# sede-open/openMCMC

Hardware: AMD Instinct MI355X
Metric: chain-updates/sec (1024 chains, 10k-node GMRF) at 1/2/4/8 GPUs vs CPU ref (higher is better)
Workload: dtype f64

## Files before the change

openmcmc_amd/csrc/omc_common.h:

```cpp
#pragma once
#include <hip/hip_runtime.h>
#include <stdint.h>

#include "omcmc_hip.h"

#define OMC_LAUNCH_LOG_MAX 64
#define OMC_SWEEP_RING_MIN 64
struct omc_ctx {
  int device;
  int dev_cus;
  int64_t n_chains;
  uint64_t seed;
  int64_t chain_offset;
  hipStream_t stream;
  bool own_stream;
  long long* d_bad_chain;
  unsigned long long* d_fallbacks;
  void* d_gamma_tab;
  unsigned long long* d_handoff;
  uint32_t run_epoch;
  int run_sweeps_per_launch;
  int run_reenter;
  int run_block_sweeps;
  int run_reenter_force;
  hipEvent_t run_ev_begin, run_ev_end;
  double* long_band; size_t long_band_bytes;
  double* long_quad; size_t long_quad_bytes;
  double* workspace;
  size_t workspace_bytes;
  void* store_ws; size_t store_ws_bytes;
  double* cov_ws; size_t cov_ws_bytes;
  void* rank_ws; size_t rank_ws_bytes;
  void* blas;
  void* blas_aux;
  hipStream_t aux_stream;
  hipEvent_t ev_fork, ev_join;
  int dense_blocked_min;
  int dense_overlap;
  double* dense_factor; size_t dense_factor_bytes;
  double* dense_winv; size_t dense_winv_bytes;
  int dense_panel_old;
  int* dense_info; size_t dense_info_bytes;
  double* slice_buf; size_t slice_buf_bytes;
// ... 373 lines not shown
```

openmcmc_amd/csrc/omc_ctx.hip:

```cpp
#include <string.h>

#include <string>

#include "omc_common.h"

static thread_local std::string g_last_error;

void omc_set_error(const char* what, hipError_t e) {
  g_last_error = std::string(what) + ": " + hipGetErrorString(e);
}

void omc_set_error_text(const char* text) { g_last_error = text; }

extern "C" {

const char* omc_last_error(void) { return g_last_error.c_str(); }

int32_t omc_abi_version(void) { return 2; }

omc_status omc_ctx_create(int32_t device, int64_t n_chains, uint64_t seed, int64_t chain_id_offset,
                          void* stream, int32_t create_stream, omc_ctx** out) {
  if (!out || n_chains <= 0 || chain_id_offset < 0) return OMC_INVALID_ARG;
  *out = nullptr;
  int count = 0;
// ... 35 lines not shown
  c->blas_aux = nullptr;
  c->aux_stream = nullptr;
  c->ev_fork = c->ev_join = nullptr;
  c->dense_overlap = 1;
  c->dense_blocked_min = 144;
  c->debug_zero_z = 0;
  c->dense_use_rocsolver = 0;
  c->gram_use_rocblas = 0;
  c->mh_use_rocblas = 0;
  c->mh_gemm_ksplit = 4;
  c->diag_algo = 0;
  c->hist_algo = 0;
  c->hist2d_algo = 0;
  c->rank_tile = 0; c->rank_chunk = 0;
  c->band_algo = 0; c->band_seg_overlap = 192; c->band_seg_count = 0; c->band_blocked_threads = 0;
  if (c->own_stream) {
    hipError_t e = hipStreamCreateWithFlags(&c->stream, hipStreamNonBlocking);
    if (e != hipSuccess) { omc_set_error("hipStreamCreate", e); delete c; return OMC_HIP_ERROR; }
  } else {
    c->stream = (hipStream_t)stream;
  }
  c->d_gamma_tab = nullptr;
  c->run_ev_begin = c->run_ev_end = nullptr;
  c->d_handoff = nullptr; c->run_epoch = 1; c->run_sweeps_per_launch = 32; c->run_reenter = 2; c->run_reenter_force = 0; c->run_block_sweeps = 0;
  hipError_t e = hipMalloc(&c->d_bad_chain, 8 * sizeof(long long));
  if (e != hipSuccess) { omc_set_error("hipMalloc", e); delete c; return OMC_HIP_ERROR; }
  c->d_fallbacks = (unsigned long long*)(c->d_bad_chain + 1);
  long long init[8] = {OMC_NO_BAD_CHAIN, 0, 0, 0, 0, 0, 0, 0};
  e = hipMemcpy(c->d_bad_chain, init, sizeof(init), hipMemcpyHostToDevice);
  if (e != hipSuccess) { omc_set_error("hipMemcpy", e); hipFree(c->d_bad_chain); delete c; return OMC_HIP_ERROR; }
  *out = c;
  return OMC_OK;
}

omc_status omc_ctx_destroy(omc_ctx* ctx) {
  if (!ctx) return OMC_INVALID_ARG;
  hipSetDevice(ctx->device);
  hipStreamSynchronize(ctx->stream);
  if (ctx->workspace) hipFree(ctx->workspace);
  if (ctx->store_ws) hipFree(ctx->store_ws);
  if (ctx->cov_ws) hipFree(ctx->cov_ws);
  if (ctx->rank_ws) hipFree(ctx->rank_ws);
  if (ctx->long_band) hipFree(ctx->long_band);
  if (ctx->long_quad) hipFree(ctx->long_quad);
  if (ctx->d_gamma_tab) hipFree(ctx->d_gamma_tab);
  if (ctx->d_handoff) hipFree(ctx->d_handoff);
  if (ctx->dense_factor) hipFree(ctx->dense_factor);
  if (ctx->dense_winv) hipFree(ctx->dense_winv);
  if (ctx->dense_info) hipFree(ctx->dense_info);
  if (ctx->slice_buf) hipFree(ctx->slice_buf);
  if (ctx->dense_tmp) hipFree(ctx->dense_tmp);
  if (ctx->rj_tmp) hipFree(ctx->rj_tmp);
  if (ctx->mh_work) hipFree(ctx->mh_work);
  if (ctx->mala.prep) hipFree(ctx->mala.prep);
  if (ctx->white.prep) hipFree(ctx->white.prep);
  if (ctx->white.a) hipFree(ctx->white.a);
  if (ctx->white.traj) hipFree(ctx->white.traj);
  if (ctx->rww.a) hipFree(ctx->rww.a);
  if (ctx->rww.mu_neg) hipFree(ctx->rww.mu_neg);
  if (ctx->rw.prep) hipFree(ctx->rw.prep);
  omc_dense_release(ctx);
  hipFree(ctx->d_bad_chain);
  if (ctx->own_stream) hipStreamDestroy(ctx->stream);
  delete ctx;
  return OMC_OK;
}

omc_status omc_ctx_synchronize(omc_ctx* ctx) {
  if (!ctx) return OMC_INVALID_ARG;
// ... 44 lines not shown
  }
  if (!strcmp(name, "band_join_fallbacks")) {
    unsigned long long v = 0;
    OMC_HIP_CHECK(hipMemcpyAsync(&v, ctx->d_fallbacks + 2, sizeof(v), hipMemcpyDeviceToHost, ctx->stream));
    OMC_HIP_CHECK(hipStreamSynchronize(ctx->stream));
    *value = (int64_t)v;
    return OMC_OK;
  }
  if (!strcmp(name, "wall_clock_khz")) {
    int khz = 0;
    OMC_HIP_CHECK(hipDeviceGetAttribute(&khz, hipDeviceAttributeWallClockRate, ctx->device));
    *value = khz;
    return OMC_OK;
  }
  if (!strcmp(name, "reenter_abi_ok")) {
    OMC_HIP_CHECK(hipSetDevice(ctx->device));
    *value = omc_reentry_probe_result(ctx);
    return OMC_OK;
  }
  if (!strcmp(name, "sweep_times_pos")) {
    *value = ctx->sweep_times_pos;
    return OMC_OK;
  }
  if (!strcmp(name, "tridiag_join_fallbacks")) {
    unsigned long long v = 0;
    OMC_HIP_CHECK(hipMemcpyAsync(&v, ctx->d_fallbacks, sizeof(v), hipMemcpyDeviceToHost, ctx->stream));
    OMC_HIP_CHECK(hipStreamSynchronize(ctx->stream));
    *value = (int64_t)v;
    return OMC_OK;
  }
  return OMC_INVALID_ARG;
}

omc_status omc_ctx_launch_log(omc_ctx* ctx, double* out, int64_t cap, int64_t* n_launches) {
  if (!ctx || !n_launches || cap < 0 || (cap > 0 && !out)) return OMC_INVALID_ARG;
  *n_launches = ctx->launch_log_total;
  const int64_t m = ctx->launch_log_n < cap ? ctx->launch_log_n : cap;
  for (int64_t i = 0; i < m; ++i) {
    const omc_ctx::LaunchRec& r = ctx->launch_log[i];
    out[5 * i] = r.t_begin; out[5 * i + 1] = r.t_end; out[5 * i + 2] = (double)r.n_sweeps; out[5 * i + 3] = (double)r.form;
    out[5 * i + 4] = (double)r.ring_pos;
  }
  return OMC_OK;
}

omc_status omc_ctx_set_option(omc_ctx* ctx, const char* name, int64_t value) {
// ... 23 lines not shown
    ctx->run_reenter = (int)value;
    ctx->run_reenter_force = 1;
    return OMC_OK;
  }
  if (!strcmp(name, "tridiag_quad_skip")) {
    if (value < 0 || value > 15) return OMC_INVALID_ARG;
    ctx->tridiag_quad_skip = (int)value;
    return OMC_OK;
  }
  if (!strcmp(name, "tridiag_perturb_ppb")) {
    if (value < 0 || value > 1000000000) return OMC_INVALID_ARG;
    ctx->tridiag_perturb_ppb = (int)value;
    return OMC_OK;
  }
  if (!strcmp(name, "tridiag_newton_max")) {
    if (value < 0 || value > 64) return OMC_INVALID_ARG;
    ctx->tridiag_newton_max = (int)value;
    return OMC_OK;
  }
  if (!strcmp(name, "tridiag_generic")) {
    ctx->tridiag_generic = value != 0;
    return OMC_OK;
  }
  if (!strcmp(name, "band_algo")) {
    if (value < 0 || value > 3) return OMC_INVALID_ARG;
    ctx->band_algo = (int)value;
    return OMC_OK;
  }
  if (!strcmp(name, "diag_algo")) {
    if (value < 0 || value > 2) return OMC_INVALID_ARG;
    ctx->diag_algo = (int)value;
    return OMC_OK;
  }
  if (!strcmp(name, "hist_algo")) {
    if (value < 0 || value > 1) return OMC_INVALID_ARG;
    ctx->hist_algo = (int)value;
    return OMC_OK;
  }
  if (!strcmp(name, "hist2d_algo")) {
    if (value < 0 || value > 3) return OMC_INVALID_ARG;
    ctx->hist2d_algo = (int)value;
    return OMC_OK;
  }
  if (!strcmp(name, "rank_tile")) {
    if (value != 0 && (value < 64 || value > 8192 || (value & (value - 1)))) return OMC_INVALID_ARG;
    ctx->rank_tile = (int)value;
// ... 84 lines not shown
```

openmcmc_amd/csrc/omc_tridiag.hip:

```cpp
#include <math.h>
#include <time.h>

#include "omc_common.h"
#include "omc_tridiag_args.h"
#include "omc_tridiag_epilogue.h"

__global__ void __launch_bounds__(64) k_tridiag_serial(TriArgs A) {
  const int64_t c = (int64_t)blockIdx.x * blockDim.x + threadIdx.x;
  if (c >= A.C) return;
  const int nt = A.T.n_terms;
  const int64_t n = A.n;
  double sc[OMC_MAX_TERMS];
  _Pragma("unroll") for (int k = 0; k < OMC_MAX_TERMS; ++k) if (k < nt) sc[k] = A.T.scale[k] ? A.T.scale[k][c] : 1.0;
  double* lw = A.work + c * n;
  double* xo = A.x + c * A.ld_x;
  const int64_t gc = A.chain_offset + c;
  bool bad = false;
  double lp = 0.0, bprev = 0.0, u = 0.0, logdet = 0.0, zodd = 0.0;
  for (int64_t i = 0; i < n; ++i) {
    double av = 0.0, bv = 0.0, rv = 0.0;
    _Pragma("unroll") for (int k = 0; k < OMC_MAX_TERMS; ++k) if (k < nt) {
      av = fma(sc[k], A.T.diag[k] ? A.T.diag[k][i] : 1.0, av);
      if (A.T.off[k] && i < n - 1) bv = fma(sc[k], A.T.off[k][i], bv);
      if (A.T.rhs[k]) rv = fma(sc[k], A.T.rhs[k][i], rv);
// ... 73 lines not shown
  const bool no_private = private_size == 0u && (rsrc2 & 1u) == 0u && (props & (1u << 11)) == 0u;
  const bool wave64 = (props & (1u << 10)) == 0u;
  return user_sgprs && system_sgprs && no_private && wave64 && preload == 0u;
}

static int g_reentry_ok = -1;
static bool reentry_abi_ok(omc_ctx* ctx) {
  if (g_reentry_ok >= 0) return g_reentry_ok != 0;
  uint32_t* d = nullptr;
  uint32_t h[6] = {~0u, ~0u, ~0u, ~0u, ~0u, ~0u};
  bool ok = hipMalloc(&d, sizeof(h)) == hipSuccess;
  if (ok) {
    hipLaunchKernelGGL(k_reentry_probe, dim3(1), dim3(64), 0, ctx->stream, d);
    ok = hipMemcpyAsync(h, d, sizeof(h), hipMemcpyDeviceToHost, ctx->stream) == hipSuccess &&
         hipStreamSynchronize(ctx->stream) == hipSuccess;
    hipFree(d);
  }
  ok = ok && reentry_descriptor_ok(h[0], h[1], h[2]) && reentry_descriptor_ok(h[3], h[4], h[5]);
  g_reentry_ok = ok ? 1 : 0;
  if (!ok) omc_set_error_text("omc_gmrf_run: the kernel descriptor does not match the restart's entry state; self-restarting workgroups are off");
  return ok;
}
int omc_reentry_probe_result(omc_ctx* ctx) { return reentry_abi_ok(ctx) ? 1 : 0; }

__global__ void k_tridiag_matvec(int64_t n, const double* diag, const double* off, const double* v, double* out) {
  for (int64_t i = (int64_t)blockIdx.x * blockDim.x + threadIdx.x; i < n; i += (int64_t)gridDim.x * blockDim.x) {
    double t = (diag ? diag[i] : 1.0) * v[i];
    if (off) {
      if (i > 0) t = fma(off[i - 1], v[i - 1], t);
      if (i < n - 1) t = fma(off[i], v[i + 1], t);
    }
    out[i] = t;
  }
}

__global__ void __launch_bounds__(256) k_tridiag_matvec_chain(int64_t n, const double* diag, const double* off, const double* v,
                                                              int64_t ld_v, const double* scale, double* out, int64_t ld_o,
                                                              int accumulate) {
  const int64_t c = blockIdx.y;
  const double s = scale ? scale[c] : 1.0;
  const double* vc = v + c * ld_v;
  for (int64_t i = (int64_t)blockIdx.x * blockDim.x + threadIdx.x; i < n; i += (int64_t)gridDim.x * blockDim.x) {
    double t = (diag ? diag[i] : 1.0) * vc[i];
    if (off) {
      if (i > 0) t = fma(off[i - 1], vc[i - 1], t);
      if (i < n - 1) t = fma(off[i], vc[i + 1], t);
// ... 132 lines not shown
    const bool on = k < t->n_terms;
    d->diag[k] = on ? t->diag[k] : nullptr;
    d->off[k] = on ? t->off[k] : nullptr;
    d->rhs[k] = on ? t->rhs[k] : nullptr;
    d->center[k] = on ? t->center[k] : nullptr;
    d->scale[k] = on ? t->scale[k] : nullptr;
  }
  if (cc) {
    *cc = CentreChain{};
    for (int k = 0; k < t->n_terms; ++k)
      if (t->center_chain[k]) {
        cc->k = cc->v ? -1 : k;
        cc->v = t->center_chain[k];
      }
    cc->ld = t->ld_center_chain;
  }
  return true;
}
static bool has_center_chain(const CentreChain& cc) { return cc.v != nullptr; }

static void args_defaults(omc_ctx* ctx, TriArgs* A, int64_t n) {
  A->T = TermsDev{};
  A->cc = CentreChain{};
  A->n = n; A->C = ctx->n_chains; A->chain_offset = ctx->chain_offset;
  A->rhs_chain = nullptr; A->ld_rhs = 0;
  A->z = nullptr; A->ld_z = 0; A->zero_z = 0;
  A->key = omc_make_key(ctx->seed, 0, OMC_RNG_NORMAL);
  A->x = nullptr; A->ld_x = 0; A->quad = nullptr; A->logdet = nullptr;
  A->bad = ctx->d_bad_chain;
  A->fallbacks = ctx->d_fallbacks;
  A->newton_max = ctx->tridiag_newton_max;
  A->perturb_start = ctx->tridiag_perturb_ppb * 1e-9;
  A->work = nullptr;
  A->fused = 0;
  A->stamps = ctx->stamps;
  A->sweep_times = nullptr; A->sweep_times_cap = 0; A->sweep_times_pos = 0;
  A->log_post = nullptr;
  A->gb_dev = nullptr; A->gdraw_dev = nullptr;
  A->n_sweeps = 0; A->reenter = 0; A->block_sweeps = 0; A->early_draws = 0; A->epoch = 0; A->seed = ctx->seed; A->handoff = nullptr; A->timeouts = ctx->d_fallbacks + 1;
  for (int k = 0; k < OMC_MAX_TERMS; ++k) A->gdraw[k] = 0;
  for (int i = 0; i < OMC_RUN_MAX; ++i) { A->rec[i].draw = 0; A->rec[i].x = nullptr; A->rec[i].log_post = nullptr; A->rec[i].slot_off = -1; }
  for (int k = 0; k < OMC_MAX_TERMS; ++k) {
    A->gb[k].enabled = 0; A->gb[k].a0 = A->gb[k].b0 = A->gb[k].half_npos = A->gb[k].lnorm = 0.0;
    A->gb[k].g_inject = nullptr; A->gb[k].store = nullptr; A->gb[k].scale_out = nullptr;
    A->gb[k].logdet_unscaled = nullptr; A->gb[k].key = A->key;
  }
// ... 327 lines not shown
    if (!ctx->d_handoff) {
      const size_t bytes = (size_t)C * OMC_HANDOFF_WORDS * sizeof(unsigned long long);
      OMC_HIP_CHECK(hipMalloc(&ctx->d_handoff, bytes));
      OMC_HIP_CHECK(hipMemsetAsync(ctx->d_handoff, 0, bytes, ctx->stream));
      ctx->run_epoch = 1;
    }
    A.handoff = ctx->d_handoff;
    A.ld_x = ld_x;
    A.zero_z = ctx->debug_zero_z;
    A.fused = 1;
    const int per = ctx->run_sweeps_per_launch < OMC_RUN_MAX ? ctx->run_sweeps_per_launch : OMC_RUN_MAX;
    const int dev_cus = ctx->dev_cus;
    const int64_t rounds = (C + dev_cus - 1) / dev_cus;
    const bool whole_rounds = C >= dev_cus && (double)C >= 0.95 * (double)(rounds * dev_cus);
    A.reenter = (whole_rounds || ctx->run_reenter_force) ? ctx->run_reenter : 0;
    if (!takes_specialised(ctx, A.T, n) || has_center_chain(A.cc)) A.reenter = 0;
    if (A.reenter && per > 1 && !reentry_abi_ok(ctx)) A.reenter = 0;
    if (A.reenter && C * (int64_t)per >= ((int64_t)1 << 26)) A.reenter = 0;
    A.early_draws = (A.reenter == 0 && 2 * C <= dev_cus && !has_center_chain(A.cc)) ? 1 : 0;
    const int64_t stored_per_launch_max = (A.reenter == 0 && n_slots < per) ? n_slots : per;
    ctx->launch_log_n = 0; ctx->launch_log_total = 0;
    const bool clock_on = ctx->sweep_times && ctx->sweep_times_cap >= OMC_SWEEP_RING_MIN;
    if (ctx->run_ev_begin) OMC_HIP_CHECK(hipEventRecord(ctx->run_ev_begin, ctx->stream));
    for (int64_t t0 = 0; t0 < total;) {
      int k_sw = (int)(total - t0 < per ? total - t0 : per);
      if (stored_per_launch_max < per) {
        int64_t stored_seen = 0;
        for (int i = 0; i < k_sw; ++i) {
          const int64_t t = t0 + i;
          if (t >= burn && ((t - burn + 1) % n_thin == 0) && ++stored_seen > stored_per_launch_max) { k_sw = i; break; }
        }
      }
      for (int i = 0; i < k_sw; ++i) {
        const int64_t t = t0 + i;
        const bool stored = t >= burn && ((t - burn + 1) % n_thin == 0);
        const int64_t it = stored ? (t - burn + 1) / n_thin - 1 : 0;
        const int64_t slot = (first_slot + it) % n_slots;
        A.rec[i].draw = draw_index0 + (uint64_t)t * draws_per_sweep;
        A.rec[i].x = stored ? x_store + slot * x_slot_stride : (t == total - 1 ? scratch_x : nullptr);
        A.rec[i].log_post = (stored && log_post_store) ? log_post_store + slot * C : nullptr;
        A.rec[i].slot_off = stored ? slot * C : -1;
      }
      A.n_sweeps = k_sw;
      A.block_sweeps = k_sw;
      if (A.reenter && ctx->run_block_sweeps > 0 && ctx->run_block_sweeps < k_sw) A.block_sweeps = ctx->run_block_sweeps;
      A.epoch = ctx->run_epoch;
      ctx->run_epoch += (uint32_t)k_sw;
      A.key = omc_make_key(ctx->seed, A.rec[0].draw, OMC_RNG_NORMAL);
      A.x = A.rec[0].x;
      A.log_post = A.rec[0].log_post;
      if (clock_on) {
        A.sweep_times = ctx->sweep_times; A.sweep_times_cap = ctx->sweep_times_cap; A.sweep_times_pos = ctx->sweep_times_pos;
      }
      const double t_begin = omc_host_clock();
      omc_status st = launch_tridiag(ctx, A);
      if (st != OMC_OK) return st;
      if (ctx->launch_log_n < OMC_LAUNCH_LOG_MAX) {
        omc_ctx::LaunchRec& r = ctx->launch_log[ctx->launch_log_n++];
        r.t_begin = t_begin; r.t_end = omc_host_clock(); r.n_sweeps = k_sw; r.form = A.reenter;
        r.ring_pos = clock_on ? ctx->sweep_times_pos : -1;
      }
      ctx->launch_log_total++;
      if (clock_on) ctx->sweep_times_pos = (ctx->sweep_times_pos + k_sw) % ctx->sweep_times_cap;
      t0 += k_sw;
    }
    if (ctx->run_ev_end) OMC_HIP_CHECK(hipEventRecord(ctx->run_ev_end, ctx->stream));
    return OMC_OK;
  }
  ctx->launch_log_n = 0; ctx->launch_log_total = 0;
  for (int64_t t = 0; t < total; ++t) {
    const bool stored = t >= burn && ((t - burn + 1) % n_thin == 0);
    const int64_t i = stored ? (t - burn + 1) / n_thin - 1 : 0;
    const int64_t slot = (first_slot + i) % n_slots;
    const uint64_t base = draw_index0 + (uint64_t)t * draws_per_sweep;
    for (int k = 0; k < terms->n_terms && k < OMC_MAX_TERMS; ++k) {
      b[k] = blocks[k];
      b[k].draw_index = base + blocks[k].draw_index;
      b[k].store = (stored && blocks[k].store) ? blocks[k].store + slot * C : nullptr;
    }
    const double t_begin = omc_host_clock();
    omc_status st = omc_gmrf_sweep(ctx, n, terms, b, nullptr, 0, nullptr, 0, base,
                                   stored ? x_store + slot * x_slot_stride : scratch_x, ld_x,
                                   (stored && log_post_store) ? log_post_store + slot * C : nullptr);
    if (st != OMC_OK) return st;
    if (ctx->launch_log_n < OMC_LAUNCH_LOG_MAX) {
      omc_ctx::LaunchRec& r = ctx->launch_log[ctx->launch_log_n++];
      r.t_begin = t_begin; r.t_end = omc_host_clock(); r.n_sweeps = 1; r.form = 0; r.ring_pos = -1;
    }
    ctx->launch_log_total++;
  }
  return OMC_OK;
}
// ... 77 lines not shown
```

openmcmc_amd/csrc/omc_tridiag_args.h:

```cpp
#pragma once
#include "omc_common.h"

struct TermsDev {
  int n_terms;
  const double* diag[OMC_MAX_TERMS];
  const double* off[OMC_MAX_TERMS];
  const double* rhs[OMC_MAX_TERMS];
  const double* center[OMC_MAX_TERMS];
  const double* scale[OMC_MAX_TERMS];
};
struct CentreChain {
  const double* v;
  int64_t ld;
  int quad_skip;
  int k;
};

struct GammaDev {
  int enabled;
  double a0, b0, half_npos;
  double lnorm;
  const double* g_inject;
  double* store;
  double* scale_out;
// ... 24 lines not shown
  double perturb_start;
  int newton_max;
  unsigned long long* fallbacks;
  double* work;
  unsigned long long* stamps;
  int fused;
  GammaDev gb[OMC_MAX_TERMS];
  const GammaDev* gb_dev;
  const unsigned long long* gdraw_dev;
  double* log_post;
  int n_sweeps;
  int reenter;
  int block_sweeps;
  int early_draws;
  uint32_t epoch;
  uint64_t seed;
  uint64_t gdraw[OMC_MAX_TERMS];
  unsigned long long* handoff;
  unsigned long long* timeouts;
  unsigned long long* sweep_times;
  int64_t sweep_times_cap, sweep_times_pos;
  SweepRec rec[OMC_RUN_MAX];
  CentreChain cc;
};

__device__ __forceinline__ bool run_mode(const TriArgs& A) { return A.n_sweeps > 0; }
__device__ __forceinline__ omc_rng_key sweep_gamma_key(const TriArgs& A, int sw, const GammaDev& g, uint64_t gd) {
  return run_mode(A) ? omc_make_key(A.seed, A.rec[sw].draw + gd, OMC_RNG_GAMMA) : g.key;
}
__device__ __forceinline__ double* sweep_gamma_store(const TriArgs& A, int sw, const GammaDev& g) {
  if (!run_mode(A)) return g.store;
  const int64_t off = A.rec[sw].slot_off;
  return (g.store && off >= 0) ? g.store + off : nullptr;
}
__device__ __forceinline__ double* sweep_log_post(const TriArgs& A, int sw) { return run_mode(A) ? A.rec[sw].log_post : A.log_post; }
```

openmcmc_amd/csrc/omc_tridiag_seg.h:

```cpp
#pragma once
#include "omc_tridiag_epilogue.h"
#include "omc_tridiag_scan.h"
#include "omc_tridiag_tile.h"

#ifndef OMC_PARK_OFF
#define OMC_PARK_OFF 1
#endif
#ifndef OMC_PARK_DIAG
#define OMC_PARK_DIAG 1
#endif
#ifndef OMC_SHIFT_PARK_C
#define OMC_SHIFT_PARK_C 1
#endif
#ifndef OMC_PREFETCH_QUAD
#define OMC_PREFETCH_QUAD 1
#endif
#ifndef OMC_WHATIF_NOSTORE
#define OMC_WHATIF_NOSTORE 0
#endif
#ifndef OMC_WHATIF_NOQLOAD
#define OMC_WHATIF_NOQLOAD 0
#endif
#ifndef OMC_NO_STAMPS
#define OMC_NO_STAMPS 0
// ... 74 lines not shown
    }
    c = blk;
    s = threadIdx.x;
    geo.chain0 = c;
  } else {
    const int cpw = 64 / G;
    geo.chain0 = ((int64_t)blockIdx.x * nw + wave) * cpw;
    c = geo.chain0 + lane / G;
    s = lane % G;
  }
  double* tile = lds_tile[wave];
  const double* trow = tile + (MULTI ? lane : s) * (M + 1);
  double* crow = tile + lane * (M + 1);
  const int lbase = TileMap<M>::lane_base(lane);
  const int pos = MULTI ? lane : s;
  const bool chain_ok = c < A.C;
  const int64_t cc = chain_ok ? c : 0;
  const int64_t n = A.n;
  const int64_t i0 = (int64_t)s * M;
  const int nt = (SMO) ? 2 : A.T.n_terms;
  const int wave_u = __builtin_amdgcn_readfirstlane(wave);
  const int r0 = TM::lane_col(lane);
  double* tl = tile + lbase;

  double sc[OMC_MAX_TERMS];
  const bool handed = MULTI && sw > 0;
  const bool hand_lds = SIG == 1 && A.reenter != 0 && restarted;
  if (SIG == 1 && A.reenter != 0 && !restarted && threadIdx.x < 2 * OMC_MAX_TERMS)
    __hip_atomic_store(lds_hand + threadIdx.x, 0ull, __ATOMIC_RELAXED, __HIP_MEMORY_SCOPE_WORKGROUP);
  unsigned long long hw[2 * OMC_MAX_TERMS];
  auto load_hand_global = [&](int k) __attribute__((always_inline)) {
    const unsigned long long* h = A.handoff + cc * OMC_HANDOFF_WORDS + 2 * k;
    hw[2 * k] = __hip_atomic_load(h, __ATOMIC_RELAXED, __HIP_MEMORY_SCOPE_AGENT);
    hw[2 * k + 1] = __hip_atomic_load(h + 1, __ATOMIC_RELAXED, __HIP_MEMORY_SCOPE_AGENT);
  };
  auto load_hand_lds = [&](int k) __attribute__((always_inline)) {
    hw[2 * k] = __hip_atomic_load(lds_hand + 2 * k, __ATOMIC_RELAXED, __HIP_MEMORY_SCOPE_WORKGROUP);
    hw[2 * k + 1] = __hip_atomic_load(lds_hand + 2 * k + 1, __ATOMIC_RELAXED, __HIP_MEMORY_SCOPE_WORKGROUP);
  };
#pragma unroll
  for (int k = 0; k < OMC_MAX_TERMS; ++k) {
    sc[k] = 1.0;
    hw[2 * k] = hw[2 * k + 1] = 0ull;
    if (k < nt && A.T.scale[k]) {
      if (handed && A.gb[k].enabled) {
        if (!hand_lds) load_hand_global(k);
// ... 87 lines not shown
    bool f = false;
    const double g = sweep_gamma_draws_wave<MULTI && !SMO>(A, c, lane, &f, sw);
    lds_g[lane] = f ? -g : g;
  }

  OMC_STAMP(1);
  const int64_t gc = A.chain_offset + cc;
  const uint32_t blk0 = (uint32_t)(i0 >> 1);
  const bool gen_z = !A.z && !A.zero_z;
  auto park_pair = [&](int jb) __attribute__((always_inline)) {
    double z0, z1;
    omc_normal_pair(omc_rng_block(nkey_f(), gc, blk0 + (uint32_t)jb), z0, z1);
    lds_z[wave][2 * jb][lane] = z0;
    lds_z[wave][2 * jb + 1][lane] = z1;
  };
  auto park_pair_over_load = [&](int jb, double (&v)[M], const double* base, int nvalid) __attribute__((always_inline)) {
    double z0, z1;
    if (nvalid == 64 * M) draws_over_load<M, true>(nkey_f(), gc, blk0 + (uint32_t)jb, z0, z1, v, base, lane, nvalid);
    else draws_over_load<M, false>(nkey_f(), gc, blk0 + (uint32_t)jb, z0, z1, v, base, lane, nvalid);
    lds_z[wave][2 * jb][lane] = z0;
    lds_z[wave][2 * jb + 1][lane] = z1;
  };
  const double* const vPark = (SHIFT && OMC_SHIFT_PARK_C) ? vSh : vPo;
  const bool park_off = OMC_PARK_OFF && SMO && gen_z && (A.quad || A.fused) &&
                        wave_valid<M>(wave_u, (int)n - ((SHIFT && OMC_SHIFT_PARK_C) ? 0 : 1)) == 64 * M &&
                        (reinterpret_cast<uintptr_t>(vPark) & 15u) == 0;
  const bool park_diag = OMC_PARK_DIAG && SMO && (A.quad || A.fused) && wave_valid<M>(wave_u, (int)n) == 64 * M &&
                         (reinterpret_cast<uintptr_t>(vPd) & 15u) == 0;
  const int e_nv = EARLY ? wave_valid<M>(wave_u, (int)n) : 0, e_nvo = EARLY ? wave_valid<M>(wave_u, (int)n - 1) : 0;
  const bool e_partial = EARLY && (A.quad || A.fused) && e_nv > 0 && e_nv < 64 * M && !(A.rhs_chain && chain_ok);
  const bool park_off_p = OMC_PARK_OFF && e_partial && gen_z && e_nvo >= 2 && (reinterpret_cast<uintptr_t>(vPo) & 15u) == 0;
  double e_edge_o = 0.0;

  const bool early1 = !EARLY && SMO && gen_z && A.early_draws != 0;
  const bool gen_late = gen_z && !EARLY && !early1;
  if constexpr (SMO && !EARLY) {
    if (early1) {
#pragma unroll
      for (int jb = 0; jb < NZB; ++jb) park_pair(jb);
    }
  }
  double pre[M];
  double Rrow[EARLY ? M : 1], ebm1_raw = 0.0, ezl0 = 0.0, ezl1 = 0.0;
  if constexpr (EARLY) {
    if (gen_z) {
#pragma unroll
      for (int jb = 0; jb < NZB; ++jb) park_pair(jb);
    }
    if (epi_wave && chain_ok) {
      bool f = false;
      const double g = sweep_gamma_draws_wave(A, c, lane, &f, sw);
// ... 16 lines not shown
      wave_lds_fence();
    };
    if (!(A.rhs_chain && chain_ok)) {
      stage(vIr + wbase, env);
#pragma unroll
      for (int j = 0; j < M; ++j) Rrow[j] = crow[j];
    }
    stage(vPo + wbase, envo);
#pragma unroll
    for (int j = 0; j < M; ++j) Y[j] = crow[j];
    stage(vPd + wbase, env);
    __builtin_amdgcn_sched_barrier(0);
    if (handed) {
      if (threadIdx.x < 2 * OMC_MAX_TERMS) __hip_atomic_store(lds_hand + threadIdx.x, 0ull, __ATOMIC_RELAXED, __HIP_MEMORY_SCOPE_WORKGROUP);
      lds_barrier();
    }
  }
  auto fill_draws = [&](int jb) {
    if constexpr (PARKZ && !SMO) {
      if (gen_z && jb < NZB) park_pair(jb);
    }
  };
  double bm1 = 0.0;
  if constexpr (SMO) {
    const int wbase = wave_u * 64 * M;
    const int nv = wave_valid<M>(wave_u, (int)n), nvo = wave_valid<M>(wave_u, (int)n - 1);
    auto vec_and_draws = [&](double (&v)[M], const double* base, int nvalid, int jb) {
      if (gen_late && jb < NZB) park_pair_over_load(jb, v, base, nvalid);
      else coal_load<M>(v, base, lane, nvalid);
      __builtin_amdgcn_sched_barrier(0);
    };
    {
      double po[M];
      double bm1_raw;
      if constexpr (EARLY) {
        bm1_raw = ebm1_raw;
      } else {
        bm1_raw = vPo[(i0 > 0 && i0 < n) ? i0 - 1 : 0];
        vec_and_draws(po, vPo + wbase, nvo, 0);
      }
      take_scales();
      if (SIG == 1 && A.reenter == 2 && handed && hand_lds && wave_u == 1 && chain_ok && any_handed_f()) {
        double* const lp_prev = A.rec[sw - 1].log_post;
        if (lp_prev) {
          const int k = lane >> 4;
          const double sk = (k == 0) ? sc[0] : ((k == 1) ? sc[1] : ((k == 2) ? sc[2] : sc[3]));
          const double qk = (k < nt) ? __hip_atomic_load(lds_q + (k < nt ? k : 0), __ATOMIC_RELAXED, __HIP_MEMORY_SCOPE_WORKGROUP) : 0.0;
          double ldk = 0.0;
          _Pragma("unroll") for (int t = 0; t < OMC_MAX_TERMS; ++t)
            if (t < nt && k == t && A.gb[t].logdet_unscaled) ldk = A.gb[t].logdet_unscaled[0];
          sweep_log_post_wave(A, c, lane, (k < nt) ? sk : 1.0, qk, ldk, lp_prev);
        }
      }
      sP = p_first ? sc[0] : sc[1];
      sI = p_first ? sc[1] : sc[0];
      if constexpr (EARLY) {
#pragma unroll
        for (int j = 0; j < M; ++j) Y[j] *= sP;
        if (!(A.rhs_chain && chain_ok)) {
#pragma unroll
          for (int j = 0; j < M; ++j) Rrow[j] *= sI;
        }
      } else {
        wave_lds_fence();
#pragma unroll
        for (int t = 0; t < M; ++t) *TM::elem(tl, r0, t) = sP * po[t];
        wave_lds_fence();
      }
      bm1 = (i0 > 0 && i0 < n) ? sP * bm1_raw : 0.0;
    }
    if constexpr (EARLY) {
      OMC_STAMP(2);
    } else {
      double pd[M];
      vec_and_draws(pd, vPd + wbase, nv, 1);
#pragma unroll
      for (int j = 0; j < M; ++j) Y[j] = crow[j];
      OMC_STAMP(2);
      wave_lds_fence();
      if (nv == 64 * M) {
#pragma unroll
        for (int t = 0; t < M; ++t) *TM::elem(tl, r0, t) = fma(sP, pd[t], sI);
      } else {
#pragma unroll
        for (int t = 0; t < M; ++t) *TM::elem(tl, r0, t) = (lane + 64 * t < nv) ? fma(sP, pd[t], sI) : 1.0;
      }
      wave_lds_fence();
    }
  } else {
    take_scales();
    if (MULTI) tile_fill_comb_wg<M, COMB_OFF>(tile, lane, wave, lbase, A, sc, chain_ok, cc, [&](int b) { if (b == 0) fill_draws(0); });
    else tile_fill_comb<M, MULTI, COMB_OFF>(tile, geo, A, sc);
#pragma unroll
    for (int j = 0; j < M; ++j) Y[j] = crow[j];
    if (i0 > 0 && i0 < n)
      _Pragma("unroll") for (int k = 0; k < OMC_MAX_TERMS; ++k) if (k < nt)
        if (A.T.off[k]) bm1 = fma(sc[k], A.T.off[k][i0 - 1], bm1);
    OMC_STAMP(2);
    if (MULTI) tile_fill_comb_wg<M, COMB_DIAG>(tile, lane, wave, lbase, A, sc, chain_ok, cc, [&](int b) { if (b == 0) fill_draws(1); });
    else tile_fill_comb<M, MULTI, COMB_DIAG>(tile, geo, A, sc);
  }
  const double* arow = crow;
  auto a_at = [&](int j) -> double {
    if constexpr (EARLY) return fma(sP, arow[j], sI);
    else return arow[j];
  };

  OMC_STAMP(3);
  double Dst;
  double Dnext0 = 0.0;
  {
    Mob m{1.0, 0.0, 0.0, 1.0};
    double bp = bm1;
#pragma unroll
    for (int j = 0; j < M; ++j) {
      const double b2 = bp * bp, aj = a_at(j);
      const double na = fma(aj, m.a, -b2 * m.c), nb = fma(aj, m.b, -b2 * m.d);
      m.c = m.a; m.d = m.b; m.a = na; m.b = nb;
      bp = Y[j];
      if ((j & 7) == 7) {
        const int ex = -__builtin_amdgcn_frexp_exp(m.a);
        m = Mob{ldexp(m.a, ex), ldexp(m.b, ex), ldexp(m.c, ex), ldexp(m.d, ex)};
      }
    }
    m = mob_rescale(m);
    OMC_STAMP(4);
    const Mob idm{1.0, 0.0, 0.0, 1.0};
    const Mob E = MULTI ? excl_scan_wg<Mob, false, true>(m, idm, lds_mob, lane, wave, nw, lds_mob2)
                        : excl_scan<Mob, false>(m, idm, pos, Wd, false, lds_mob, wave, nw);
    Dst = (E.a + E.b) / (E.c + E.d);
    if (A.perturb_start != 0.0 && s > 0) Dst *= 1.0 + A.perturb_start;
    if (MULTI) {
      const Mob inc = compose(m, E);
      Dnext0 = (inc.a + inc.b) * fast_rcp(inc.c + inc.d);
      if (A.perturb_start != 0.0) Dnext0 *= 1.0 + A.perturb_start;
    }
  }

  OMC_STAMP(5);
  bool bad = false;
  double lin = 0.0;
  auto pivot_pass = [&]() -> double {
    wave_lds_fence();
    const double rst = fast_rcp(Dst);
    lin = bm1 * rst;
    double lp = lin, bprev = bm1, Dend = Dst;
    bool badp = false;
#pragma unroll
    for (int j = 0; j < M; ++j) {
      const double D = fma(-lp, bprev, a_at(j));
      badp |= !(D > 0.0);
      const double r = fast_rcp(D);
      W[j] = r;
      bprev = Y[j];
      lp = bprev * r;
      Dend = D;
    }
    bad = badp;
    return Dend;
  };
  double Dend = pivot_pass();
  bool settled = false;
  if (MULTI) {
    const bool has_next = i0 + M < n;
    const int need = (has_next && fabs(Dend - Dnext0) > OMC_NEWTON_TOL * fabs(Dnext0)) ? 1 : 0;
    settled = !any_wg(need, lds_any, lane, wave, nw);
  }
  for (int it = 0; !settled; ++it) {
    double J = lin * lin;
#pragma unroll
    for (int j = 0; j + 1 < M; ++j) {
      const double l = Y[j] * W[j];
      J *= l * l;
    }
    double Dp = Dend, Jp = J;
    if (MULTI) prev_lane2_wg(Dp, Jp, Dst, 0.0, lds_x[it & 1], lane, wave, nw);
    else prev_lane2<false>(Dp, Jp, Dst, 0.0, pos, Wd, lds_x[0], wave);
    const bool joined = (s > 0 && i0 < n);
    const double e = joined ? (Dp - Dst) : 0.0;
    if (!joined) Jp = 0.0;
    const int need = (fabs(e) > OMC_NEWTON_TOL * fabs(Dst)) ? 1 : 0;
    const int any = MULTI ? __syncthreads_or(need) : (__ballot(need) != 0ull);
// ... 82 lines not shown
    }
  }
  if (rhs_done) {
  } else if (MULTI) {
    if constexpr (SMO) tile_fill_comb_wg<M, COMB_RHS, false>(tile, lane, wave, lbase, A, sc, chain_ok, cc);
    else tile_fill_comb_wg<M, COMB_RHS, true>(tile, lane, wave, lbase, A, sc, chain_ok, cc, [&](int b) { fill_draws(2 + b); });
    if constexpr (EARLY) {
#pragma unroll
      for (int j = 0; j < M; ++j) Rrow[j] = crow[j];
    }
  } else {
    tile_fill_comb<M, MULTI, COMB_RHS>(tile, geo, A, sc);
  }
  constexpr bool PFQ = SMO && OMC_PREFETCH_QUAD;
  constexpr int PFQ_LOADS = M;
  static_assert(!PFQ || PFQ_LOADS <= 15, "vmcnt immediate");
  double qcp[PFQ ? M : 1];
  double qcc[SHIFT ? M : 1];
  bool pfq = false;
  int pfq_behind = 0;
  auto issue_pfq = [&]() {
    if constexpr (PFQ) {
      const bool wq = A.quad || A.fused;
      pfq = wq && park_off && wave_valid<M>(wave_u, (int)n) == 64 * M;
      __builtin_amdgcn_sched_barrier(0);
      if constexpr (EARLY) {
        if (e_partial) {
          const int wbase = wave_u * 64 * M;
#pragma unroll
          for (int t = 0; t < M; ++t) qcp[t] = (lane + 64 * t < e_nv) ? (vIc + wbase)[(unsigned)(lane + 64 * t)] : 0.0;
        }
      }
      if (pfq) {
        const int wbase = wave_u * 64 * M;
        if (!SHIFT || vIc) {
#pragma unroll
          for (int t = 0; t < M; ++t) qcp[t] = (vIc + wbase)[(unsigned)(lane + 64 * t)];
          pfq_behind += M;
        } else {
#pragma unroll
          for (int t = 0; t < M; ++t) qcp[t] = 0.0;
        }
      }
      __builtin_amdgcn_sched_barrier(0);
    }
  };
  OMC_STAMP(8);
// ... 49 lines not shown
          }
        }
        if constexpr (EARLY) {
          z0 = crow[M]; z1 = ezl1;
        } else {
          omc_normal_pair(omc_rng_block(nkey_f(), gc, blk0 + (uint32_t)(j >> 1)), z0, z1);
        }
      }
      u = fma(-lp, u, r_at(j));
      W[j] = fma(u, W[j], z0 * fast_sqrt(W[j]));
      lp = Y[j];
      u = fma(-lp, u, r_at(j + 1));
      W[j + 1] = fma(u, W[j + 1], z1 * fast_sqrt(W[j + 1]));
      lp = Y[j + 1];
      if (!(PARKZ && (j >> 1) < NZB - 1)) __builtin_amdgcn_sched_barrier(0);
    }
  }

  OMC_STAMP(10);
  const bool want_quad = A.quad || A.fused;
  double aPd = 0.0;
  double eqd[EARLY ? M : 1];
  const bool diag_staged = EARLY && !(A.rhs_chain && chain_ok);
  if constexpr (SMO) {
    if (park_diag && !diag_staged) {
      lds_reads_done();
#pragma unroll
      for (int k = 0; k < (64 * M) / 128; ++k)
        __builtin_amdgcn_global_load_lds((const __attribute__((address_space(1))) void*)(vPd + wave_u * 64 * M + 128 * k + 2 * lane),
                                         (__attribute__((address_space(3))) void*)(tile + 128 * k), 16, 0, 0);
    }
  }
  issue_pfq();
  double xnext;
  {
    Aff f{0.0, 1.0};
#pragma unroll
    for (int j = M - 1; j >= 0; --j) {
      f.p = fma(-Y[j], f.p, W[j]);
      f.q = -Y[j] * f.q;
    }
    xnext = (MULTI ? excl_scan_wg<Aff, true>(f, Aff{0.0, 1.0}, lds_aff[3], lane, wave, nw)
                   : excl_scan<Aff, false>(f, Aff{0.0, 1.0}, pos, Wd, true, lds_aff[0], wave, nw)).p;
    double x = xnext;
    OMC_STAMP(11);
    if constexpr (EARLY) {
      if (e_partial) {
        wave_lds_fence();
#pragma unroll
        for (int t = 0; t < M; ++t) eqd[t] = *TM::elem(tl, r0, t);
      }
    }
    if (SMO && park_diag) {
      if (!diag_staged) {
        if (PFQ && pfq_behind >= PFQ_LOADS) __builtin_amdgcn_s_waitcnt(0x0F70 | PFQ_LOADS);
        else __builtin_amdgcn_s_waitcnt(0x0F70);
      }
      wave_lds_fence();
      const double* drow = diag_staged ? crow : tile + lane * M;
#pragma unroll
      for (int j = M - 1; j >= 0; --j) {
        x = fma(-Y[j], x, W[j]);
        W[j] = x;
        aPd = fma(drow[j] * x, x, aPd);
      }
    } else {
#pragma unroll
      for (int j = M - 1; j >= 0; --j) {
        x = fma(-Y[j], x, W[j]);
        W[j] = x;
      }
    }
  }
  OMC_STAMP(12);
  double qsum[OMC_MAX_TERMS] = {0, 0, 0, 0};
  double my_scale = 1.0, my_logdet = 0.0;
  if (MULTI) {
    wave_lds_fence();
#pragma unroll
    for (int j = 0; j < M; ++j) crow[j] = W[j];
    if (lane == 63) tile[64 * (M + 1)] = xnext;
    wave_lds_fence();
    double acc[OMC_MAX_TERMS] = {0, 0, 0, 0};
    if (epi_wave) {
      _Pragma("unroll") for (int k = 0; k < OMC_MAX_TERMS; ++k) if (k < nt && (lane >> 4) == k) {
        if (A.T.scale[k]) my_scale = handed ? sc[k] : A.T.scale[k][cc];
        if constexpr (SMO) {
          if (sweep_log_post(A, sw) && A.gb[k].logdet_unscaled) my_logdet = A.gb[k].logdet_unscaled[0];
        }
      }
      if constexpr (!SMO) {
        const double* const ldp = ((lane >> 4) < nt) ? A.gb_dev[lane >> 4].logdet_unscaled : nullptr;
        if (sweep_log_post(A, sw) && ldp) my_logdet = ldp[0];
      }
    }
    if constexpr (SMO) {
      if (!EARLY && epi_wave && chain_ok) {
        bool f = false;
        const double g = sweep_gamma_draws_wave(A, c, lane, &f, sw);
        lds_g[lane] = f ? -g : g;
      }
      const int nv = wave_valid<M>(wave_u, (int)n);
      double qc[M], qd[M], qo[M];
      {
        const int wbase = wave_u * 64 * M;
        const int nvq = want_quad ? nv : 0, nvo = want_quad ? wave_valid<M>(wave_u, (int)n - 1) : 0;
        {
          if (park_off && SHIFT && OMC_SHIFT_PARK_C) {
            const double* zf = &lds_z[wave][0][0];
            coal_load<M>(qo, vPo + wbase, lane, nvo);
            __builtin_amdgcn_s_waitcnt(0x0F70 | M);
            wave_lds_fence();
#pragma unroll
            for (int t = 0; t < M; ++t)
              if (t < 2 * NZB) qcc[t] = zf[64 * t + lane];
#pragma unroll
            for (int t = 0; t < M; ++t) {
              if (t < 2 * NZB) continue;
              qcc[t] = (vSh + wbase)[(unsigned)(lane + 64 * t)];
            }
          } else if (park_off) {
            const double* zf = &lds_z[wave][0][0];
            __builtin_amdgcn_s_waitcnt(0x0F70);
            wave_lds_fence();
#pragma unroll
            for (int t = 0; t < M; ++t)
              if (t < 2 * NZB) qo[t] = zf[64 * t + lane];
#pragma unroll
            for (int t = 0; t < M; ++t) {
              if (t < 2 * NZB) continue;
              qo[t] = OMC_WHATIF_NOQLOAD ? 0.25 : (vPo + wbase)[(unsigned)(lane + 64 * t)];
// ... 217 lines not shown
```

Measured before the change: 13.08 million.

## Detect constant tridiagonal slices and skip per-element diag/off loads

Adds a pre-pass kernel that checks whether each wave-sized slice of the precision diagonal and off-diagonal is constant, and records the flags and values in a small table. In the specialised single-term segment kernel, waves whose slice is constant use the scalar value instead of loading the vector from global memory or staging it through LDS. This targets memory traffic and LDS work in the factor and quad passes. The cost is an extra launch per run plus added branches and register pressure, and the fast path only applies when the inputs happen to have constant runs.

Result: no change. 13.21 million, median of 6 (+0.9%).

```diff
diff --git a/openmcmc_amd/csrc/omc_common.h b/openmcmc_amd/csrc/omc_common.h
--- a/openmcmc_amd/csrc/omc_common.h
+++ b/openmcmc_amd/csrc/omc_common.h
@@ -5,6 +5,10 @@
 #include "omcmc_hip.h"
 
 #define OMC_LAUNCH_LOG_MAX 64
+#define OMC_SLICE_WORDS 4
+#define OMC_SLICE_MAX 16
+#define OMC_SLICE_OFF 1ull
+#define OMC_SLICE_DIAG 2ull
 #define OMC_SWEEP_RING_MIN 64
 struct omc_ctx {
   int device;
@@ -19,6 +23,9 @@
   void* d_gamma_tab;
   unsigned long long* d_handoff;
   uint32_t run_epoch;
+  unsigned long long* d_slices;
+  int run_slices;
+  int run_slices_n;
   int run_sweeps_per_launch;
   int run_reenter;
   int run_block_sweeps;
diff --git a/openmcmc_amd/csrc/omc_ctx.hip b/openmcmc_amd/csrc/omc_ctx.hip
--- a/openmcmc_amd/csrc/omc_ctx.hip
+++ b/openmcmc_amd/csrc/omc_ctx.hip
@@ -81,6 +81,7 @@
   }
   c->d_gamma_tab = nullptr;
   c->run_ev_begin = c->run_ev_end = nullptr;
+  c->d_slices = nullptr; c->run_slices = 1; c->run_slices_n = 0;
   c->d_handoff = nullptr; c->run_epoch = 1; c->run_sweeps_per_launch = 32; c->run_reenter = 2; c->run_reenter_force = 0; c->run_block_sweeps = 0;
   hipError_t e = hipMalloc(&c->d_bad_chain, 8 * sizeof(long long));
   if (e != hipSuccess) { omc_set_error("hipMalloc", e); delete c; return OMC_HIP_ERROR; }
@@ -104,6 +105,7 @@
   if (ctx->long_quad) hipFree(ctx->long_quad);
   if (ctx->d_gamma_tab) hipFree(ctx->d_gamma_tab);
   if (ctx->d_handoff) hipFree(ctx->d_handoff);
+  if (ctx->d_slices) hipFree(ctx->d_slices);
   if (ctx->dense_factor) hipFree(ctx->dense_factor);
   if (ctx->dense_winv) hipFree(ctx->dense_winv);
   if (ctx->dense_info) hipFree(ctx->dense_info);
@@ -194,6 +196,17 @@
     *value = ctx->sweep_times_pos;
     return OMC_OK;
   }
+  if (!strcmp(name, "tridiag_const_slices")) {
+    unsigned long long w[OMC_SLICE_MAX * OMC_SLICE_WORDS];
+    const int m = ctx->run_slices_n;
+    *value = 0;
+    if (m <= 0 || !ctx->d_slices) return OMC_OK;
+    OMC_HIP_CHECK(hipMemcpyAsync(w, ctx->d_slices, (size_t)m * OMC_SLICE_WORDS * sizeof(w[0]), hipMemcpyDeviceToHost, ctx->stream));
+    OMC_HIP_CHECK(hipStreamSynchronize(ctx->stream));
+    for (int i = 0; i < m; ++i)
+      *value += (int64_t)((w[OMC_SLICE_WORDS * i] & OMC_SLICE_OFF) != 0ull) + (int64_t)((w[OMC_SLICE_WORDS * i] & OMC_SLICE_DIAG) != 0ull);
+    return OMC_OK;
+  }
   if (!strcmp(name, "tridiag_join_fallbacks")) {
     unsigned long long v = 0;
     OMC_HIP_CHECK(hipMemcpyAsync(&v, ctx->d_fallbacks, sizeof(v), hipMemcpyDeviceToHost, ctx->stream));
@@ -263,6 +276,10 @@
     ctx->tridiag_generic = value != 0;
     return OMC_OK;
   }
+  if (!strcmp(name, "tridiag_slices")) {
+    ctx->run_slices = value != 0;
+    return OMC_OK;
+  }
   if (!strcmp(name, "band_algo")) {
     if (value < 0 || value > 3) return OMC_INVALID_ARG;
     ctx->band_algo = (int)value;
diff --git a/openmcmc_amd/csrc/omc_tridiag.hip b/openmcmc_amd/csrc/omc_tridiag.hip
--- a/openmcmc_amd/csrc/omc_tridiag.hip
+++ b/openmcmc_amd/csrc/omc_tridiag.hip
@@ -119,6 +119,29 @@
   return ok;
 }
 int omc_reentry_probe_result(omc_ctx* ctx) { return reentry_abi_ok(ctx) ? 1 : 0; }
+
+__global__ void __launch_bounds__(256) k_tridiag_slices(int64_t n, int slice, const double* diag, const double* off,
+                                                        unsigned long long* tab) {
+  const int64_t base = (int64_t)blockIdx.x * slice;
+  const bool in_d = base + slice <= n, in_o = base + slice <= n - 1;
+  const unsigned long long* const d = reinterpret_cast<const unsigned long long*>(diag) + base;
+  const unsigned long long* const o = reinterpret_cast<const unsigned long long*>(off) + base;
+  const unsigned long long d0 = in_d ? d[0] : 0ull, o0 = in_o ? o[0] : 0ull;
+  int same_d = in_d ? 1 : 0, same_o = in_o ? 1 : 0;
+  for (int i = threadIdx.x; i < slice; i += blockDim.x) {
+    if (in_d) same_d &= (d[i] == d0) ? 1 : 0;
+    if (in_o) same_o &= (o[i] == o0) ? 1 : 0;
+  }
+  same_d = __syncthreads_and(same_d);
+  same_o = __syncthreads_and(same_o);
+  if (threadIdx.x == 0) {
+    unsigned long long* const e = tab + (int64_t)blockIdx.x * OMC_SLICE_WORDS;
+    e[0] = (same_o ? OMC_SLICE_OFF : 0ull) | (same_d ? OMC_SLICE_DIAG : 0ull);
+    e[1] = o0;
+    e[2] = d0;
+    e[3] = 0ull;
+  }
+}
 
 __global__ void k_tridiag_matvec(int64_t n, const double* diag, const double* off, const double* v, double* out) {
   for (int64_t i = (int64_t)blockIdx.x * blockDim.x + threadIdx.x; i < n; i += (int64_t)gridDim.x * blockDim.x) {
@@ -297,6 +320,7 @@
 static void args_defaults(omc_ctx* ctx, TriArgs* A, int64_t n) {
   A->T = TermsDev{};
   A->cc = CentreChain{};
+  A->slices = nullptr;
   A->n = n; A->C = ctx->n_chains; A->chain_offset = ctx->chain_offset;
   A->rhs_chain = nullptr; A->ld_rhs = 0;
   A->z = nullptr; A->ld_z = 0; A->zero_z = 0;
@@ -670,6 +694,21 @@
     ctx->launch_log_n = 0; ctx->launch_log_total = 0;
     const bool clock_on = ctx->sweep_times && ctx->sweep_times_cap >= OMC_SWEEP_RING_MIN;
     if (ctx->run_ev_begin) OMC_HIP_CHECK(hipEventRecord(ctx->run_ev_begin, ctx->stream));
+    ctx->run_slices_n = 0;
+    if (ctx->run_slices && total >= 2 && takes_specialised(ctx, A.T, n) && !has_center_chain(A.cc) &&
+        !(A.early_draws && !A.reenter && !A.zero_z)) {
+      const int seg = ctx->tridiag_seg ? ctx->tridiag_seg : auto_seg(n);
+      const int n_sl = (int)((n + 64 * seg - 1) / (64 * seg));
+      if (n_sl <= OMC_SLICE_MAX) {
+        if (!ctx->d_slices) OMC_HIP_CHECK(hipMalloc(&ctx->d_slices, (size_t)OMC_SLICE_MAX * OMC_SLICE_WORDS * sizeof(unsigned long long)));
+        const bool p_first = A.T.diag[0] != nullptr;
+        hipLaunchKernelGGL(k_tridiag_slices, dim3((unsigned)n_sl), dim3(256), 0, ctx->stream, n, 64 * seg,
+                           p_first ? A.T.diag[0] : A.T.diag[1], p_first ? A.T.off[0] : A.T.off[1], ctx->d_slices);
+        OMC_HIP_CHECK(hipGetLastError());
+        A.slices = ctx->d_slices;
+        ctx->run_slices_n = n_sl;
+      }
+    }
     for (int64_t t0 = 0; t0 < total;) {
       int k_sw = (int)(total - t0 < per ? total - t0 : per);
       if (stored_per_launch_max < per) {
@@ -716,6 +755,7 @@
     return OMC_OK;
   }
   ctx->launch_log_n = 0; ctx->launch_log_total = 0;
+  ctx->run_slices_n = 0;
   for (int64_t t = 0; t < total; ++t) {
     const bool stored = t >= burn && ((t - burn + 1) % n_thin == 0);
     const int64_t i = stored ? (t - burn + 1) / n_thin - 1 : 0;
diff --git a/openmcmc_amd/csrc/omc_tridiag_args.h b/openmcmc_amd/csrc/omc_tridiag_args.h
--- a/openmcmc_amd/csrc/omc_tridiag_args.h
+++ b/openmcmc_amd/csrc/omc_tridiag_args.h
@@ -70,6 +70,7 @@
   int64_t sweep_times_cap, sweep_times_pos;
   SweepRec rec[OMC_RUN_MAX];
   CentreChain cc;
+  const unsigned long long* slices;
 };
 
 __device__ __forceinline__ bool run_mode(const TriArgs& A) { return A.n_sweeps > 0; }
diff --git a/openmcmc_amd/csrc/omc_tridiag_seg.h b/openmcmc_amd/csrc/omc_tridiag_seg.h
--- a/openmcmc_amd/csrc/omc_tridiag_seg.h
+++ b/openmcmc_amd/csrc/omc_tridiag_seg.h
@@ -1,4 +1,6 @@
 #pragma once
+#include <type_traits>
+
 #include "omc_tridiag_epilogue.h"
 #include "omc_tridiag_scan.h"
 #include "omc_tridiag_tile.h"
@@ -120,6 +122,16 @@
   const int wave_u = __builtin_amdgcn_readfirstlane(wave);
   const int r0 = TM::lane_col(lane);
   double* tl = tile + lbase;
+  unsigned long long sl_flags = 0ull;
+  double off0 = 0.0, d0 = 0.0;
+  if constexpr (SIG == 1) {
+    if (A.slices) {
+      const auto* st = (const __attribute__((address_space(4))) unsigned long long*)(uintptr_t)A.slices + OMC_SLICE_WORDS * wave_u;
+      sl_flags = st[0];
+      off0 = __longlong_as_double((long long)st[1]);
+      d0 = __longlong_as_double((long long)st[2]);
+    }
+  }
 
   double sc[OMC_MAX_TERMS];
   const bool handed = MULTI && sw > 0;
@@ -253,11 +265,14 @@
     lds_z[wave][2 * jb + 1][lane] = z1;
   };
   const double* const vPark = (SHIFT && OMC_SHIFT_PARK_C) ? vSh : vPo;
-  const bool park_off = OMC_PARK_OFF && SMO && gen_z && (A.quad || A.fused) &&
-                        wave_valid<M>(wave_u, (int)n - ((SHIFT && OMC_SHIFT_PARK_C) ? 0 : 1)) == 64 * M &&
-                        (reinterpret_cast<uintptr_t>(vPark) & 15u) == 0;
+  const bool c_off = SIG == 1 && (sl_flags & OMC_SLICE_OFF) != 0ull && wave_valid<M>(wave_u, (int)n - 1) == 64 * M;
+  const bool park_off_any = OMC_PARK_OFF && SMO && gen_z && (A.quad || A.fused) &&
+                            wave_valid<M>(wave_u, (int)n - ((SHIFT && OMC_SHIFT_PARK_C) ? 0 : 1)) == 64 * M &&
+                            (reinterpret_cast<uintptr_t>(vPark) & 15u) == 0;
+  const bool park_off = park_off_any && !c_off;
   const bool park_diag = OMC_PARK_DIAG && SMO && (A.quad || A.fused) && wave_valid<M>(wave_u, (int)n) == 64 * M &&
                          (reinterpret_cast<uintptr_t>(vPd) & 15u) == 0;
+  const bool c_diag = SIG == 1 && (sl_flags & OMC_SLICE_DIAG) != 0ull && park_diag;
   const int e_nv = EARLY ? wave_valid<M>(wave_u, (int)n) : 0, e_nvo = EARLY ? wave_valid<M>(wave_u, (int)n - 1) : 0;
   const bool e_partial = EARLY && (A.quad || A.fused) && e_nv > 0 && e_nv < 64 * M && !(A.rhs_chain && chain_ok);
   const bool park_off_p = OMC_PARK_OFF && e_partial && gen_z && e_nvo >= 2 && (reinterpret_cast<uintptr_t>(vPo) & 15u) == 0;
@@ -320,12 +335,17 @@
     }
   };
   double bm1 = 0.0;
+  double a0 = 0.0;
   if constexpr (SMO) {
     const int wbase = wave_u * 64 * M;
     const int nv = wave_valid<M>(wave_u, (int)n), nvo = wave_valid<M>(wave_u, (int)n - 1);
     auto vec_and_draws = [&](double (&v)[M], const double* base, int nvalid, int jb) {
       if (gen_late && jb < NZB) park_pair_over_load(jb, v, base, nvalid);
       else coal_load<M>(v, base, lane, nvalid);
+      __builtin_amdgcn_sched_barrier(0);
+    };
+    auto draws_alone = [&](int jb) {
+      if (gen_late && jb < NZB) park_pair(jb);
       __builtin_amdgcn_sched_barrier(0);
     };
     {
@@ -359,7 +379,7 @@
 #pragma unroll
           for (int j = 0; j < M; ++j) Rrow[j] *= sI;
         }
-      } else {
+      } else if (!c_off) {
         wave_lds_fence();
 #pragma unroll
         for (int t = 0; t < M; ++t) *TM::elem(tl, r0, t) = sP * po[t];
@@ -371,12 +391,20 @@
       OMC_STAMP(2);
     } else {
       double pd[M];
-      vec_and_draws(pd, vPd + wbase, nv, 1);
-#pragma unroll
-      for (int j = 0; j < M; ++j) Y[j] = crow[j];
+      if (c_diag) draws_alone(1);
+      else vec_and_draws(pd, vPd + wbase, nv, 1);
+      if (c_off) {
+#pragma unroll
+        for (int j = 0; j < M; ++j) Y[j] = sP * off0;
+      } else {
+#pragma unroll
+        for (int j = 0; j < M; ++j) Y[j] = crow[j];
+      }
       OMC_STAMP(2);
       wave_lds_fence();
-      if (nv == 64 * M) {
+      if (c_diag) {
+        a0 = fma(sP, d0, sI);
+      } else if (nv == 64 * M) {
 #pragma unroll
         for (int t = 0; t < M; ++t) *TM::elem(tl, r0, t) = fma(sP, pd[t], sI);
       } else {
@@ -399,28 +427,40 @@
     else tile_fill_comb<M, MULTI, COMB_DIAG>(tile, geo, A, sc);
   }
   const double* arow = crow;
-  auto a_at = [&](int j) -> double {
-    if constexpr (EARLY) return fma(sP, arow[j], sI);
+  auto a_at = [&](int j, auto cd) -> double {
+    if constexpr (decltype(cd)::value) return a0;
+    else if constexpr (EARLY) return fma(sP, arow[j], sI);
     else return arow[j];
+  };
+  using CdYes = std::integral_constant<bool, true>;
+  using CdNo = std::integral_constant<bool, false>;
+  auto by_diag = [&](auto f) {
+    if constexpr (SIG == 1) {
+      if (c_diag) return f(CdYes{});
+    }
+    return f(CdNo{});
   };
 
   OMC_STAMP(3);
   double Dst;
   double Dnext0 = 0.0;
   {
-    Mob m{1.0, 0.0, 0.0, 1.0};
-    double bp = bm1;
-#pragma unroll
-    for (int j = 0; j < M; ++j) {
-      const double b2 = bp * bp, aj = a_at(j);
-      const double na = fma(aj, m.a, -b2 * m.c), nb = fma(aj, m.b, -b2 * m.d);
-      m.c = m.a; m.d = m.b; m.a = na; m.b = nb;
-      bp = Y[j];
-      if ((j & 7) == 7) {
-        const int ex = -__builtin_amdgcn_frexp_exp(m.a);
-        m = Mob{ldexp(m.a, ex), ldexp(m.b, ex), ldexp(m.c, ex), ldexp(m.d, ex)};
-      }
-    }
+    Mob m = by_diag([&](auto cd) {
+      Mob m{1.0, 0.0, 0.0, 1.0};
+      double bp = bm1;
+#pragma unroll
+      for (int j = 0; j < M; ++j) {
+        const double b2 = bp * bp, aj = a_at(j, cd);
+        const double na = fma(aj, m.a, -b2 * m.c), nb = fma(aj, m.b, -b2 * m.d);
+        m.c = m.a; m.d = m.b; m.a = na; m.b = nb;
+        bp = Y[j];
+        if ((j & 7) == 7) {
+          const int ex = -__builtin_amdgcn_frexp_exp(m.a);
+          m = Mob{ldexp(m.a, ex), ldexp(m.b, ex), ldexp(m.c, ex), ldexp(m.d, ex)};
+        }
+      }
+      return m;
+    });
     m = mob_rescale(m);
     OMC_STAMP(4);
     const Mob idm{1.0, 0.0, 0.0, 1.0};
@@ -442,20 +482,22 @@
     wave_lds_fence();
     const double rst = fast_rcp(Dst);
     lin = bm1 * rst;
-    double lp = lin, bprev = bm1, Dend = Dst;
-    bool badp = false;
-#pragma unroll
-    for (int j = 0; j < M; ++j) {
-      const double D = fma(-lp, bprev, a_at(j));
-      badp |= !(D > 0.0);
-      const double r = fast_rcp(D);
-      W[j] = r;
-      bprev = Y[j];
-      lp = bprev * r;
-      Dend = D;
-    }
-    bad = badp;
-    return Dend;
+    return by_diag([&](auto cd) {
+      double lp = lin, bprev = bm1, Dend = Dst;
+      bool badp = false;
+#pragma unroll
+      for (int j = 0; j < M; ++j) {
+        const double D = fma(-lp, bprev, a_at(j, cd));
+        badp |= !(D > 0.0);
+        const double r = fast_rcp(D);
+        W[j] = r;
+        bprev = Y[j];
+        lp = bprev * r;
+        Dend = D;
+      }
+      bad = badp;
+      return Dend;
+    });
   };
   double Dend = pivot_pass();
   bool settled = false;
@@ -584,7 +626,7 @@
   auto issue_pfq = [&]() {
     if constexpr (PFQ) {
       const bool wq = A.quad || A.fused;
-      pfq = wq && park_off && wave_valid<M>(wave_u, (int)n) == 64 * M;
+      pfq = wq && park_off_any && wave_valid<M>(wave_u, (int)n) == 64 * M;
       __builtin_amdgcn_sched_barrier(0);
       if constexpr (EARLY) {
         if (e_partial) {
@@ -680,13 +722,15 @@
   double aPd = 0.0;
   double eqd[EARLY ? M : 1];
   const bool diag_staged = EARLY && !(A.rhs_chain && chain_ok);
+  int diag_xfers = 0;
   if constexpr (SMO) {
-    if (park_diag && !diag_staged) {
+    if (park_diag && !diag_staged && !c_diag) {
       lds_reads_done();
 #pragma unroll
       for (int k = 0; k < (64 * M) / 128; ++k)
         __builtin_amdgcn_global_load_lds((const __attribute__((address_space(1))) void*)(vPd + wave_u * 64 * M + 128 * k + 2 * lane),
                                          (__attribute__((address_space(3))) void*)(tile + 128 * k), 16, 0, 0);
+      diag_xfers += (64 * M) / 128;
     }
   }
   issue_pfq();
@@ -710,17 +754,26 @@
       }
     }
     if (SMO && park_diag) {
-      if (!diag_staged) {
+      if (diag_xfers > 0) {
         if (PFQ && pfq_behind >= PFQ_LOADS) __builtin_amdgcn_s_waitcnt(0x0F70 | PFQ_LOADS);
         else __builtin_amdgcn_s_waitcnt(0x0F70);
       }
       wave_lds_fence();
-      const double* drow = diag_staged ? crow : tile + lane * M;
-#pragma unroll
-      for (int j = M - 1; j >= 0; --j) {
-        x = fma(-Y[j], x, W[j]);
-        W[j] = x;
-        aPd = fma(drow[j] * x, x, aPd);
+      if (c_diag) {
+#pragma unroll
+        for (int j = M - 1; j >= 0; --j) {
+          x = fma(-Y[j], x, W[j]);
+          W[j] = x;
+          aPd = fma(d0 * x, x, aPd);
+        }
+      } else {
+        const double* drow = diag_staged ? crow : tile + lane * M;
+#pragma unroll
+        for (int j = M - 1; j >= 0; --j) {
+          x = fma(-Y[j], x, W[j]);
+          W[j] = x;
+          aPd = fma(drow[j] * x, x, aPd);
+        }
       }
     } else {
 #pragma unroll
@@ -764,7 +817,10 @@
         const int wbase = wave_u * 64 * M;
         const int nvq = want_quad ? nv : 0, nvo = want_quad ? wave_valid<M>(wave_u, (int)n - 1) : 0;
         {
-          if (park_off && SHIFT && OMC_SHIFT_PARK_C) {
+          if (c_off) {
+#pragma unroll
+            for (int t = 0; t < M; ++t) qo[t] = off0;
+          } else if (park_off && SHIFT && OMC_SHIFT_PARK_C) {
             const double* zf = &lds_z[wave][0][0];
             coal_load<M>(qo, vPo + wbase, lane, nvo);
             __builtin_amdgcn_s_waitcnt(0x0F70 | M);
```
